# loicmagne/tinynerf

Measured on AMD Instinct MI355X. Metric: ray-samples/sec (K-Planes training step: sampler + render fwd + bwd + Adam), higher is better.
Workload: dtype f32 (f16x2-split products)

## Files before the change

tinynerf_amd/csrc/b3_device.h:

```cpp
#pragma once
#include "tn_common.h"

namespace tn {
namespace b3 {

typedef __bf16 bf16x8 __attribute__((ext_vector_type(8)));
typedef unsigned u32x4 __attribute__((ext_vector_type(4)));
typedef float f32x16 __attribute__((ext_vector_type(16)));

struct Op { u32x4 hi, mid, lo; };

__device__ __forceinline__ void split2(float a, float b, unsigned &hi, unsigned &mid, unsigned &lo) {
    const unsigned ha = __float_as_uint(a) & 0xffff0000u, hb = __float_as_uint(b) & 0xffff0000u;
    const float ra = a - __uint_as_float(ha), rb = b - __uint_as_float(hb);
    const unsigned ma = __float_as_uint(ra) & 0xffff0000u, mb = __float_as_uint(rb) & 0xffff0000u;
    const float la = ra - __uint_as_float(ma), lb = rb - __uint_as_float(mb);
    hi = __builtin_amdgcn_perm(hb, ha, 0x07060302u);
    mid = __builtin_amdgcn_perm(mb, ma, 0x07060302u);
    lo = __builtin_amdgcn_perm(__float_as_uint(lb), __float_as_uint(la), 0x07060302u);
}

__device__ __forceinline__ Op split8(const float (&v)[8]) {
    Op o;
#pragma unroll
    for (int p = 0; p < 4; ++p) {
        unsigned a, b, c;
        split2(v[2 * p], v[2 * p + 1], a, b, c);
        o.hi[p] = a; o.mid[p] = b; o.lo[p] = c;
    }
    return o;
}

__device__ __forceinline__ f32x16 mfma16(const u32x4 &a, const u32x4 &b, f32x16 c) {
    return __builtin_amdgcn_mfma_f32_32x32x16_bf16(__builtin_bit_cast(bf16x8, a), __builtin_bit_cast(bf16x8, b), c, 0, 0, 0);
}

__device__ __forceinline__ f32x16 mfma6(const Op &A, const Op &B, f32x16 acc) {
    acc = mfma16(A.lo, B.hi, acc);
    acc = mfma16(A.hi, B.lo, acc);
    acc = mfma16(A.mid, B.mid, acc);
    acc = mfma16(A.mid, B.hi, acc);
    acc = mfma16(A.hi, B.mid, acc);
    acc = mfma16(A.hi, B.hi, acc);
    return acc;
}

}
}
```

tinynerf_amd/csrc/mlp_wgrad_rc.hip:

```cpp
#include "mlp_stage.h"
#include "mlp_f2_heads.h"
#include "b3_device.h"
#include <algorithm>

#ifndef TN_RC_SB
#define TN_RC_SB
#endif
#ifdef TN_PHASE_TIMERS
__device__ unsigned long long tn_phase_cycles_rc[16];
#define TN_PTR_BEGIN unsigned long long ptr_ = __builtin_amdgcn_s_memtime();
#define TN_PTR(k) { __builtin_amdgcn_sched_barrier(0); const unsigned long long n_ = __builtin_amdgcn_s_memtime(); if (tn::lane_id() == 0) atomicAdd(&tn_phase_cycles_rc[k], n_ - ptr_); ptr_ = __builtin_amdgcn_s_memtime(); __builtin_amdgcn_sched_barrier(0); }
extern "C" int tn_debug_phase_cycles_rc(unsigned long long *out, int reset) {
    hipMemcpyFromSymbol(out, HIP_SYMBOL(tn_phase_cycles_rc), sizeof(unsigned long long) * 16);
    if (reset) { unsigned long long z[16] = {}; hipMemcpyToSymbol(HIP_SYMBOL(tn_phase_cycles_rc), z, sizeof(z)); }
    return 0;
}
#else
#define TN_PTR_BEGIN
#define TN_PTR(k)
#endif
namespace {

using tn::f32x16;
using tn::f32x4;
using namespace tn::mlp;
namespace b3 = tn::b3;

constexpr int H = 64, NH = 4;

template <int CTRL>
__device__ __forceinline__ float dpp_max(float v) {
    return fmaxf(v, __int_as_float(__builtin_amdgcn_update_dpp(0, __float_as_int(v), CTRL, 0xf, 0xf, true)));
}
__device__ __forceinline__ float wave_max(float m) {
    m = dpp_max<0xB1>(m);
    m = dpp_max<0x4E>(m);
    m = dpp_max<0x141>(m);
    m = dpp_max<0x128>(m);
    const auto r16 = __builtin_amdgcn_permlane16_swap(__float_as_uint(m), __float_as_uint(m), false, false);
    m = fmaxf(__uint_as_float(r16[0]), __uint_as_float(r16[1]));
    const auto r32 = __builtin_amdgcn_permlane32_swap(__float_as_uint(m), __float_as_uint(m), false, false);
    return fmaxf(__uint_as_float(r32[0]), __uint_as_float(r32[1]));
}

__device__ __forceinline__ void load_block_f(const float *__restrict__ rows, int i, int h, float (&v)[16]) {
    const f32x4 *p = reinterpret_cast<const f32x4 *>(rows + i * 32 + 4 * h);
#pragma unroll
    for (int q = 0; q < 4; ++q) {
        const f32x4 t = p[2 * q];
        v[4 * q] = t[0]; v[4 * q + 1] = t[1]; v[4 * q + 2] = t[2]; v[4 * q + 3] = t[3];
    }
}

__device__ __forceinline__ void split_block(const float (&v)[16], b3::Op (&op)[2]) {
    const float a[8] = {v[0], v[1], v[2], v[3], v[4], v[5], v[6], v[7]};
    const float b[8] = {v[8], v[9], v[10], v[11], v[12], v[13], v[14], v[15]};
    op[0] = b3::split8(a);
    op[1] = b3::split8(b);
}

struct WOp { u32x4h a0h, a0l, a1h, a1l; };
__device__ __forceinline__ WOp load_w(const _Float16 *__restrict__ Wh, int plane, int stride, int j, int h, int b) {
    const _Float16 *p0 = Wh + j * stride + 16 * b + 8 * h, *p1 = p0 + 32 * stride;
    WOp w;
    w.a0h = *reinterpret_cast<const u32x4h *>(p0); w.a0l = *reinterpret_cast<const u32x4h *>(p0 + plane);
    w.a1h = *reinterpret_cast<const u32x4h *>(p1); w.a1l = *reinterpret_cast<const u32x4h *>(p1 + plane);
    return w;
}
template <bool S>
__device__ __forceinline__ void mma_sf(const WOp &w, const u32x4h &bh, const u32x4h &bl, f32x16 (&accS)[2], f32x16 (&accF)[2], bool first = false) {
    const f32x16 z = {0.f, 0.f, 0.f, 0.f, 0.f, 0.f, 0.f, 0.f, 0.f, 0.f, 0.f, 0.f, 0.f, 0.f, 0.f, 0.f};
    if constexpr (S) {
        accS[0] = mfma_f16(w.a0l, bh, first ? z : accS[0]);
        accS[1] = mfma_f16(w.a1l, bh, first ? z : accS[1]);
    }
    accF[0] = mfma_f16(bh, w.a0l, first ? z : accF[0]);
    accF[1] = mfma_f16(bh, w.a1l, first ? z : accF[1]);
    if constexpr (S) {
        accS[0] = mfma_f16(w.a0h, bl, accS[0]);
        accS[1] = mfma_f16(w.a1h, bl, accS[1]);
    }
    accF[0] = mfma_f16(bl, w.a0h, accF[0]);
    accF[1] = mfma_f16(bl, w.a1h, accF[1]);
    if constexpr (S) {
        accS[0] = mfma_f16(w.a0h, bh, accS[0]);
        accS[1] = mfma_f16(w.a1h, bh, accS[1]);
    }
    accF[0] = mfma_f16(bh, w.a0h, accF[0]);
    accF[1] = mfma_f16(bh, w.a1h, accF[1]);
}

__device__ __forceinline__ void zero2(f32x16 (&a)[2]) {
#pragma unroll
    for (int ob = 0; ob < 2; ++ob)
#pragma unroll
        for (int r = 0; r < 16; ++r) a[ob][r] = 0.0f;
}

struct RcArgs {
    MlpArgs a, b;
    const float *x, *aux;
    const float *ws_a, *ws_b;
    float *gW[5], *gB[5];
    float *gWs, *gBs;
    int64_t n;
};

template <int WPB, bool AUX, int OA, int OB, int NGA, int NBA>
__device__ __forceinline__ void wgrad_rc_body(const RcArgs &p, const float *__restrict__ ldsa, const float *__restrict__ ldsb, float *__restrict__ ,
                                              const float *__restrict__ px, const float *__restrict__ paux, const int *__restrict__ paidx,
                                              const float *__restrict__ pws_a, const float *__restrict__ pws_b)
{
    const int lane = tn::lane_id(), j_ = lane & 31, h_ = lane >> 5;
    const int wave = __builtin_amdgcn_readfirstlane(threadIdx.x >> 6);
    const int64_t n = p.n, n_tiles = (n + 31) >> 5;
    const int Rta = stash_rows(H, NH, 0), Rtb = stash_rows(H, 1, 0);
    constexpr int nga = NGA, nba = NBA;
    constexpr bool has_aux = AUX;

    f32x16 acc[3][2][2];
#pragma unroll
    for (int l = 0; l < 3; ++l)
#pragma unroll
        for (int tn_ = 0; tn_ < 2; ++tn_)
#pragma unroll
            for (int tk = 0; tk < 2; ++tk)
#pragma unroll
                for (int r = 0; r < 16; ++r) acc[l][tn_][tk][r] = 0.0f;
    float db[3][2] = {{0.f, 0.f}, {0.f, 0.f}, {0.f, 0.f}};
    float dwo[OA][2], dws[OB][2], dbo[OA], dbs[OB];
#pragma unroll
    for (int o = 0; o < OA; ++o) { dwo[o][0] = dwo[o][1] = 0.f; dbo[o] = 0.f; }
#pragma unroll
    for (int o = 0; o < OB; ++o) { dws[o][0] = dws[o][1] = 0.f; dbs[o] = 0.f; }

    f32x4 fr[12], av[8];
    auto fetch_x = [&](int64_t t) {
        int64_t r = t * 32 + j_;
        r = r < n ? r : n - 1;
        const float *xr = px + r * 96 + 4 * h_;
#pragma unroll
        for (int g = 0; g < 12; ++g) fr[g] = *reinterpret_cast<const f32x4 *>(xr + 8 * g);
    };
    int aidx = 0;
    auto fetch_aidx = [&](int64_t t) {
        int64_t r = t * 32 + j_;
        r = r < n ? r : n - 1;
        if constexpr (has_aux) aidx = paidx[r];
    };
    auto fetch_aux = [&]() {
        if constexpr (has_aux) {
            const float *arow = paux + (int64_t)aidx * p.a.aux_stride + 4 * h_;
#pragma unroll
            for (int g = 0; g < 8; ++g) av[g] = *reinterpret_cast<const f32x4 *>(arow + 8 * (g < nga ? g : nga - 1));
        }
    };
    {
        const int64_t t0 = (int64_t)blockIdx.x * WPB + wave;
        fetch_aidx(t0 < n_tiles ? t0 : n_tiles - 1);
        fetch_aux();
        fetch_x(t0 < n_tiles ? t0 : n_tiles - 1);
    }
    float gqa[2][16], gqb[2][16];
    for (int64_t tile = (int64_t)blockIdx.x * WPB + wave; tile < n_tiles; tile += (int64_t)gridDim.x * WPB) {
        int j = j_, h = h_;
        asm volatile("" : "+v"(j), "+v"(h));
        const float *wsa = pws_a + tile * (int64_t)(Rta * 32);
        const float *wsb = pws_b + tile * (int64_t)(Rtb * 32);
        const _Float16 *W0 = reinterpret_cast<const _Float16 *>(ldsa + p.a.w_off[0]);
        const int plane0 = p.a.f2_plane[0], st0 = p.a.stride[0];
        const int64_t tile_next = tile + (int64_t)gridDim.x * WPB < n_tiles ? tile + (int64_t)gridDim.x * WPB : n_tiles - 1;
        fetch_aidx(tile_next);
        TN_PTR_BEGIN

        f32x16 accS[2], accF[2], actS[2], actF[2];
        if constexpr (has_aux) {
            WOp w = load_w(W0, plane0, st0, j, h, 6);
            float m = 0.0f;
#pragma unroll
            for (int g = 0; g < 8; ++g) m = fmaxf(fmaxf(m, fmaxf(fabsf(av[g][0]), fabsf(av[g][1]))), fmaxf(fabsf(av[g][2]), fabsf(av[g][3])));
            float s_a, inv_a;
            f2_scales(wave_max(m), s_a, inv_a);
#pragma unroll
            for (int ba = 0; ba < nba; ++ba) {
                const WOp wn = load_w(W0, plane0, st0, j, h, 6 + (ba + 1 < nba ? ba + 1 : ba));
                const float v[8] = {av[2 * ba][0], av[2 * ba][1], av[2 * ba][2], av[2 * ba][3], av[2 * ba + 1][0], av[2 * ba + 1][1], av[2 * ba + 1][2], av[2 * ba + 1][3]};
                u32x4h bh, bl;
                f2_split8(v, s_a, bh, bl);
                mma_sf<true>(w, bh, bl, accS, accF, ba == 0);
                TN_RC_SB
                w = wn;
            }
            const float ca = inv_a * ldsa[p.a.f2_scale + 1];
#pragma unroll
            for (int ob = 0; ob < 2; ++ob) {
#pragma unroll
                for (int r = 0; r < 16; ++r) { actS[ob][r] = accS[ob][r] * ca; actF[ob][r] = accF[ob][r] * ca; }
            }
        } else {
            zero2(actS); zero2(actF);
        }
        TN_RC_SB
        TN_PTR(0)
        u32x4h xbh[6], xbl[6];
        float inv_x;
        {
            float m = 0.0f;
#pragma unroll
            for (int g = 0; g < 12; ++g) m = fmaxf(fmaxf(m, fmaxf(fabsf(fr[g][0]), fabsf(fr[g][1]))), fmaxf(fabsf(fr[g][2]), fabsf(fr[g][3])));
            float s_x;
            f2_scales(wave_max(m), s_x, inv_x);
#pragma unroll
            for (int b = 0; b < 6; ++b) {
                const float v[8] = {fr[2 * b][0], fr[2 * b][1], fr[2 * b][2], fr[2 * b][3], fr[2 * b + 1][0], fr[2 * b + 1][1], fr[2 * b + 1][2], fr[2 * b + 1][3]};
                f2_split8(v, s_x, xbh[b], xbl[b]);
            }
        }
        TN_RC_SB
        TN_PTR(1)
        load_block_f(wsa + (int64_t)((NH + 1) * H) * 32, j, h, gqa[0]);
        load_block_f(wsa + (int64_t)((NH + 1) * H + 32) * 32, j, h, gqa[1]);
        {
            WOp w = load_w(W0, plane0, st0, j, h, 0);
#pragma unroll
            for (int b = 0; b < 6; ++b) {
                const WOp wn = load_w(W0, plane0, st0, j, h, b + 1 < 6 ? b + 1 : b);
                mma_sf<true>(w, xbh[b], xbl[b], accS, accF, b == 0);
                TN_RC_SB
                w = wn;
            }
            const float cx = inv_x * ldsa[p.a.f2_scale + 1];
#pragma unroll
            for (int ob = 0; ob < 2; ++ob) {
                const f32x16 bias = tn::bias_tile(ldsa + p.a.b_off[0], ob, h);
                const float bl_ = ldsa[p.a.b_off[0] + 32 * ob + j];
#pragma unroll
                for (int r = 0; r < 16; ++r) {
                    actS[ob][r] = fmaf(accS[ob][r], cx, actS[ob][r]) + bias[r];
                    actF[ob][r] = fmaf(accF[ob][r], cx, actF[ob][r]) + bl_;
                }
                actS[ob] = tn::relu16(actS[ob]);
                actF[ob] = tn::relu16(actF[ob]);
            }
        }
        TN_RC_SB
        TN_PTR(2)
        {
            const _Float16 *W0s = reinterpret_cast<const _Float16 *>(ldsb + p.b.w_off[0]);
            const int pls = p.b.f2_plane[0], sts = p.b.stride[0];
            float gs[OB][16];
#pragma unroll
            for (int o = 0; o < OB; ++o) load_block_f(wsb + 2 * H * 32, o, h, gs[o]);
            WOp w = load_w(W0s, pls, sts, j, h, 0);
#pragma unroll
            for (int b = 0; b < 6; ++b) {
                const WOp wn = load_w(W0s, pls, sts, j, h, b + 1 < 6 ? b + 1 : b);
                mma_sf<false>(w, xbh[b], xbl[b], accS, accF, b == 0);
                TN_RC_SB
                w = wn;
            }
            const float c = inv_x * ldsb[p.b.f2_scale + 1];
#pragma unroll
            for (int ob = 0; ob < 2; ++ob) {
                const float bias = ldsb[p.b.b_off[0] + 32 * ob + j];
#pragma unroll
                for (int r = 0; r < 16; ++r) accF[ob][r] = fmaf(accF[ob][r], c, bias);
                accF[ob] = tn::relu16(accF[ob]);
            }
#pragma unroll
            for (int o = 0; o < OB; ++o) {
                float s0 = 0.f, s1 = 0.f, sg = 0.f;
#pragma unroll
                for (int r = 0; r < 16; ++r) { s0 = fmaf(gs[o][r], accF[0][r], s0); s1 = fmaf(gs[o][r], accF[1][r], s1); sg += gs[o][r]; }
                dws[o][0] += s0; dws[o][1] += s1; dbs[o] += sg;
            }
        }
        TN_RC_SB
        TN_PTR(3)

        float go[OA][16];
#pragma unroll
        for (int l = 1; l <= 3; ++l) {
            const _Float16 *Wl = reinterpret_cast<const _Float16 *>(ldsa + p.a.w_off[l]);
            const int plane = p.a.f2_plane[l], stride = p.a.stride[l];
            float (&gq)[2][16] = (l == 2) ? gqb : gqa;
            if (l < 3) {
                float (&gn)[2][16] = (l == 1) ? gqb : gqa;
                load_block_f(wsa + (int64_t)((NH + l + 1) * H) * 32, j, h, gn[0]);
                load_block_f(wsa + (int64_t)((NH + l + 1) * H + 32) * 32, j, h, gn[1]);
            }
            {
                b3::Op HB[2][2];
#pragma unroll
                for (int tk = 0; tk < 2; ++tk) {
                    float v[16];
#pragma unroll
                    for (int r = 0; r < 16; ++r) v[r] = actF[tk][r];
                    split_block(v, HB[tk]);
                }
#pragma unroll
                for (int tn_ = 0; tn_ < 2; ++tn_) {
                    float sg = 0.f;
#pragma unroll
                    for (int r = 0; r < 16; ++r) sg += gq[tn_][r];
                    db[l - 1][tn_] += sg;
                    b3::Op GA[2];
                    split_block(gq[tn_], GA);
#pragma unroll
                    for (int c = 0; c < 2; ++c)
#pragma unroll
                        for (int tk = 0; tk < 2; ++tk) acc[l - 1][tn_][tk] = b3::mfma6(GA[c], HB[tk][c], acc[l - 1][tn_][tk]);
                    TN_RC_SB
                }
            }
            TN_PTR(3 + l)
            if (l == 1) fetch_aux();
            if (l == 3) {
#pragma unroll
                for (int o = 0; o < OA; ++o) load_block_f(wsa + 2 * NH * H * 32, o, h, go[o]);
                fetch_x(tile_next);
            }
            WOp w = load_w(Wl, plane, stride, j, h, 0);
            float m = 0.0f;
#pragma unroll
            for (int kb = 0; kb < 2; ++kb)
#pragma unroll
                for (int r = 0; r < 16; ++r) m = fmaxf(m, actS[kb][r]);
            float s, inv;
            f2_scales(wave_max(m), s, inv);
#pragma unroll
            for (int b = 0; b < 4; ++b) {
                const WOp wn = load_w(Wl, plane, stride, j, h, b + 1 < 4 ? b + 1 : b);
                float v[8];
#pragma unroll
                for (int e = 0; e < 8; ++e) v[e] = actS[b >> 1][8 * (b & 1) + e];
                u32x4h bh, bl;
                f2_split8(v, s, bh, bl);
                if (l < 3) mma_sf<true>(w, bh, bl, accS, accF, b == 0);
                else mma_sf<false>(w, bh, bl, accS, accF, b == 0);
                TN_RC_SB
                w = wn;
            }
            const float c = inv * ldsa[p.a.f2_scale + 2 * l + 1];
#pragma unroll
            for (int ob = 0; ob < 2; ++ob) {
                const float bl_ = ldsa[p.a.b_off[l] + 32 * ob + j];
#pragma unroll
                for (int r = 0; r < 16; ++r) actF[ob][r] = fmaf(accF[ob][r], c, bl_);
                actF[ob] = tn::relu16(actF[ob]);
                if (l < 3) {
                    const f32x16 bias = tn::bias_tile(ldsa + p.a.b_off[l], ob, h);
#pragma unroll
                    for (int r = 0; r < 16; ++r) actS[ob][r] = fmaf(accS[ob][r], c, bias[r]);
                    actS[ob] = tn::relu16(actS[ob]);
                }
            }
            TN_RC_SB
            TN_PTR(6 + l)
        }
#pragma unroll
        for (int o = 0; o < OA; ++o) {
            float s0 = 0.f, s1 = 0.f, sg = 0.f;
#pragma unroll
            for (int r = 0; r < 16; ++r) { s0 = fmaf(go[o][r], actF[0][r], s0); s1 = fmaf(go[o][r], actF[1][r], s1); sg += go[o][r]; }
            dwo[o][0] += s0; dwo[o][1] += s1; dbo[o] += sg;
        }
        TN_PTR(10)
    }

    const int i = j_, h = h_;
#pragma unroll
    for (int l = 0; l < 3; ++l) {
#pragma unroll
        for (int tn_ = 0; tn_ < 2; ++tn_) {
#pragma unroll
            for (int tk = 0; tk < 2; ++tk) {
                tn::pin16(acc[l][tn_][tk]);
#pragma unroll
                for (int r = 0; r < 16; ++r) {
                    const int nn = 32 * tn_ + (r & 3) + 8 * (r >> 2) + 4 * h;
                    atomicAdd(&p.gW[l + 1][nn * H + 32 * tk + i], acc[l][tn_][tk][r]);
                }
            }
            float s = db[l][tn_];
            s += __shfl_xor(s, 32, 64);
            if (h == 0) atomicAdd(&p.gB[l + 1][32 * tn_ + i], s);
        }
    }
#pragma unroll
    for (int o = 0; o < OA; ++o) {
#pragma unroll
        for (int tk = 0; tk < 2; ++tk) {
            float s = dwo[o][tk];
            s += __shfl_xor(s, 32, 64);
            if (h == 0) atomicAdd(&p.gW[4][o * H + 32 * tk + i], s);
        }
        float s = dbo[o];
        s += __shfl_xor(s, 32, 64);
        if (lane == 0) atomicAdd(&p.gB[4][o], s);
    }
#pragma unroll
    for (int o = 0; o < OB; ++o) {
#pragma unroll
        for (int tk = 0; tk < 2; ++tk) {
            float s = dws[o][tk];
            s += __shfl_xor(s, 32, 64);
            if (h == 0) atomicAdd(&p.gWs[o * H + 32 * tk + i], s);
        }
        float s = dbs[o];
        s += __shfl_xor(s, 32, 64);
        if (lane == 0) atomicAdd(&p.gBs[o], s);
    }
}

template <int WPB, bool AUX, int OA, int OB, int NGA, int NBA>
__global__ __launch_bounds__(WPB * 64) void wgrad_rc_kernel(RcArgs p)
{
    extern __shared__ __attribute__((aligned(16))) float lds[];
    stage_weights_f2(p.a, lds);
    stage_weights_f2(p.b, lds + p.a.lds_floats);
    wgrad_rc_body<WPB, AUX, OA, OB, NGA, NBA>(p, lds, lds + p.a.lds_floats, nullptr, p.x, p.aux,
                                              p.a.aux_index, p.ws_a, p.ws_b);
}

struct FlArgs {
    const float *x, *aux;
    const int *aux_index;
    int aux_stride, pe, K0_a, K0_b;
    const float *ws_a, *ws_b;
    int rt_a, rt_b, g0_a, g0_b;
    float *gW0, *gB0, *gW0s, *gB0s;
    int64_t n;
};

constexpr int FL_RS = 36;
constexpr int FL_IN = 96, FL_AW = 56;
constexpr int FL_BUF = 128 * FL_RS + 32 * FL_IN + 32 * FL_AW;

__global__ __launch_bounds__(512) void wgrad_first_kernel(FlArgs p)
{
    extern __shared__ __attribute__((aligned(16))) float lds[];
    constexpr int NW = 8, NCH = 4;
    constexpr int g_chunks = 128 * 8, x_chunks = 32 * FL_IN / 4;
    const int lane = tn::lane_id(), i_ = lane & 31, h_ = lane >> 5;
    const int wave = __builtin_amdgcn_readfirstlane(threadIdx.x >> 6);
    const int64_t n = p.n, n_tiles = (n + 31) >> 5;
    const bool colour = wave < 5;
    const int tk = colour ? wave : wave - 5;
    f32x16 acc[2];
    float dbacc[2] = {0.f, 0.f};
#pragma unroll
    for (int m = 0; m < 2; ++m)
#pragma unroll
        for (int r = 0; r < 16; ++r) acc[m][r] = 0.0f;
    f32x4 pre[NCH];
    f32x4 preA = {0.f, 0.f, 0.f, 0.f};
    int aidx = 0;
    auto prefetch = [&](int64_t tile, int64_t tile_after) {
        const f32x4 *sa = reinterpret_cast<const f32x4 *>(p.ws_a + tile * (int64_t)p.rt_a * 32 + (int64_t)p.g0_a * 32);
        const f32x4 *sb = reinterpret_cast<const f32x4 *>(p.ws_b + tile * (int64_t)p.rt_b * 32 + (int64_t)p.g0_b * 32);
        const int64_t x0 = tile * 32 * (int64_t)FL_IN;
        const int64_t xlast = n * (int64_t)FL_IN - 4;
#pragma unroll
        for (int k = 0; k < NCH; ++k) {
            const int c = threadIdx.x + k * NW * 64;
            int64_t e = x0 + 4 * (int64_t)(c - g_chunks);
            e = e < 0 ? 0 : (e > xlast ? xlast : e);
            const f32x4 *px = reinterpret_cast<const f32x4 *>(p.x + e);
            const f32x4 *pg = c < 512 ? sa + c : sb + ((c - 512) & 511);
            pre[k] = *(c < g_chunks ? pg : px);
        }
        {
            const int s_ = (threadIdx.x >> 4) & 31, part = threadIdx.x & 15;
            preA = *reinterpret_cast<const f32x4 *>(p.aux + (int64_t)aidx * p.aux_stride + (4 * part < FL_AW ? 4 * part : 0));
            int64_t r_ = tile_after * 32 + s_;
            r_ = r_ < n ? r_ : n - 1;
            aidx = p.aux_index[r_];
        }
    };
    float *dummy = lds + 2 * FL_BUF;
    auto commit = [&](float *buf) {
        float *ldsX = buf + 128 * FL_RS, *ldsA = ldsX + 32 * FL_IN;
#pragma unroll
        for (int k = 0; k < NCH; ++k) {
            const int c = threadIdx.x + k * NW * 64;
            float *dst = c < g_chunks ? buf + (c >> 3) * FL_RS + (c & 7) * 4 : (c < g_chunks + x_chunks ? ldsX + 4 * (c - g_chunks) : dummy);
            *reinterpret_cast<f32x4 *>(dst) = pre[k];
        }
        const int s_ = threadIdx.x >> 4, part = threadIdx.x & 15;
        float *dst = 4 * part < FL_AW ? ldsA + s_ * FL_AW + 4 * part : dummy;
        *reinterpret_cast<f32x4 *>(dst) = preA;
    };
    const int64_t last = n_tiles - 1;
    int64_t tile = blockIdx.x;
    if (tile >= n_tiles) return;
    {
        int64_t r_ = tile * 32 + ((threadIdx.x >> 4) & 31);
        r_ = r_ < n ? r_ : n - 1;
        aidx = p.aux_index[r_];
    }
    {
        const int64_t t1 = tile + gridDim.x, t2 = t1 + gridDim.x;
        prefetch(tile, t1 < last ? t1 : last);
        commit(lds);
        __syncthreads();
        prefetch(t1 < last ? t1 : last, t2 < last ? t2 : last);
    }
    int cur = 0;
    for (; tile < n_tiles; tile += gridDim.x) {
        int i = i_, h = h_;
        asm volatile("" : "+v"(i), "+v"(h));
        float *buf = lds + cur * FL_BUF;
        float *nbuf = lds + (cur ^ 1) * FL_BUF;
        const int64_t t2 = tile + 2 * (int64_t)gridDim.x, t3 = t2 + gridDim.x;
        commit(nbuf);
        prefetch(t2 < last ? t2 : last, t3 < last ? t3 : last);
        const float *ldsX = buf + 128 * FL_RS, *ldsA = ldsX + 32 * FL_IN;
        {
            const int grow = colour ? 0 : 64;
            const f32x4 *g0 = reinterpret_cast<const f32x4 *>(buf + (grow + i) * FL_RS + 16 * h);
            const f32x4 *g1 = reinterpret_cast<const f32x4 *>(buf + (grow + 32 + i) * FL_RS + 16 * h);
            const int q = 32 * tk + i;
            const bool xcol = q < FL_IN;
            const int ac = q - FL_IN < FL_AW ? q - FL_IN : FL_AW - 1;
            const float *cp = xcol ? ldsX + 16 * h * FL_IN + q : ldsA + 16 * h * FL_AW + (ac < 0 ? 0 : ac);
            const int cstride = xcol ? FL_IN : FL_AW;
            float gs0 = 0.f, gs1 = 0.f;
#pragma unroll
            for (int c = 0; c < 2; ++c) {
                const f32x4 ga = g0[2 * c], gb = g0[2 * c + 1], gc = g1[2 * c], gd = g1[2 * c + 1];
                float xv[8];
#pragma unroll
                for (int u = 0; u < 8; ++u) xv[u] = cp[(8 * c + u) * cstride];
                const float v0[8] = {ga[0], ga[1], ga[2], ga[3], gb[0], gb[1], gb[2], gb[3]};
                const float v1[8] = {gc[0], gc[1], gc[2], gc[3], gd[0], gd[1], gd[2], gd[3]};
                const b3::Op XB = b3::split8(xv);
                acc[0] = b3::mfma6(b3::split8(v0), XB, acc[0]);
                acc[1] = b3::mfma6(b3::split8(v1), XB, acc[1]);
                gs0 += ((ga[0] + ga[1]) + (ga[2] + ga[3])) + ((gb[0] + gb[1]) + (gb[2] + gb[3]));
                gs1 += ((gc[0] + gc[1]) + (gc[2] + gc[3])) + ((gd[0] + gd[1]) + (gd[2] + gd[3]));
            }
            if (tk == 0) { dbacc[0] += gs0; dbacc[1] += gs1; }
        }
        __syncthreads();
        cur ^= 1;
    }
    const int i = i_, h = h_;
    const int q = 32 * tk + i;
    int col; bool ok;
    float *gW; int ldw;
    if (colour) { gW = p.gW0; ldw = p.K0_a; ok = q < FL_IN || q - FL_IN < p.pe; col = q < FL_IN ? p.pe + q : q - FL_IN; }
    else { gW = p.gW0s; ldw = p.K0_b; ok = true; col = q; }
#pragma unroll
    for (int m = 0; m < 2; ++m) {
        tn::pin16(acc[m]);
#pragma unroll
        for (int r = 0; r < 16; ++r) {
            const int nn = 32 * m + (r & 3) + 8 * (r >> 2) + 4 * h;
            if (ok) atomicAdd(&gW[(int64_t)nn * ldw + col], acc[m][r]);
        }
        if (tk == 0) {
            float s = dbacc[m];
            s += __shfl_xor(s, 32, 64);
            if (h == 0) atomicAdd(&(colour ? p.gB0 : p.gB0s)[32 * m + i], s);
        }
    }
}

}

static bool lean_pair_ok(const tn_mlp_desc *d, const tn_mlp_desc *p)
{
    const bool f2 = (d->flags & TN_MLP_F16X2) && (p->flags & TN_MLP_F16X2);
    return f2 && d->n_layers == 5 && p->n_layers == 2 && d->in_dim == 96 && p->in_dim == 96 && d->encoding == TN_ENC_AUX_CAT &&
           p->encoding == TN_ENC_NONE && d->dims[0] == 147 && d->dims[1] == 64 && d->dims[2] == 64 && d->dims[3] == 64 &&
           d->dims[4] == 64 && d->dims[5] == 3 && p->dims[0] == 96 && p->dims[1] == 64 && p->dims[2] == 1 &&
           d->aux_stride >= FL_AW && (d->aux_stride & 3) == 0;
}

extern "C" int tn_mlp_lean_supported(const tn_mlp_desc *desc, const tn_mlp_desc *partner)
{
    return desc && partner && lean_pair_ok(desc, partner);
}

static int lean_plan(RcArgs &p, const tn_mlp_desc *desc, const tn_mlp_desc *partner, const float *x, const float *aux, int64_t n,
                     float *const *gw, float *const *gb, float *const *gws, float *const *gbs, const float *ws_a, const float *ws_b)
{
    TN_REQUIRE(desc && partner && x && gw && gb && gws && gbs && ws_a && ws_b, TN_E_NULL, "tn_mlp_wgrad_lean_pair: null pointer");
    int Ha = 0, Hb = 0;
    if (int rc = plan(desc, p.a, Ha)) return rc;
    if (int rc = plan(partner, p.b, Hb)) return rc;
    TN_REQUIRE(lean_pair_ok(desc, partner), TN_E_CONFIG, "TN_MLP_LEAN: the reference's decoders (run.py:133-139) as f16x2 heads (TN_MLP_F16X2): "
                                                         "colour 147 -> 64 x 4 -> 3 on [per-ray table (51), x (96)], sigma 96 -> 64 -> 1");
    TN_REQUIRE(aux && ((uintptr_t)aux & 15) == 0 && p.a.aux_index, TN_E_NULL, "TN_MLP_LEAN: aux table (16-byte aligned) and aux_index are required");
    TN_REQUIRE((((uintptr_t)x | (uintptr_t)ws_a | (uintptr_t)ws_b) & 15) == 0, TN_E_ALIGN, "TN_MLP_LEAN: x / workspaces must be 16-byte aligned");
    if (n <= 0) return TN_OK;
    for (int l = 0; l < 5; ++l) TN_REQUIRE(gw[l] && gb[l], TN_E_NULL, "TN_MLP_LEAN: null gradient pointer");
    TN_REQUIRE(gws[0] && gbs[0] && gws[1] && gbs[1], TN_E_NULL, "TN_MLP_LEAN: null gradient pointer");
    plan_f2(p.a, 64);
    plan_f2(p.b, 64);
    TN_REQUIRE(((size_t)p.a.lds_floats + (size_t)p.b.lds_floats) * 4 <= (size_t)LDS_LIMIT_BYTES, TN_E_CONFIG, "TN_MLP_LEAN: weights do not fit LDS");
    return TN_OK;
}

extern "C" __attribute__((visibility("hidden"))) int tn_mlp_wgrad_lean_check(const tn_mlp_desc *desc, const tn_mlp_desc *partner, const float *x,
                                                                             const float *aux, int64_t n, float *const *gw, float *const *gb,
                                                                             float *const *gws, float *const *gbs, const float *ws_a,
                                                                             const float *ws_b)
{
    RcArgs p;
    return lean_plan(p, desc, partner, x, aux, n, gw, gb, gws, gbs, ws_a, ws_b);
}

extern "C" int tn_mlp_wgrad_lean_pair(const tn_mlp_desc *desc, const tn_mlp_desc *partner, const float *x, const float *aux, int64_t n,
                                      float *const *gw, float *const *gb, float *const *gws, float *const *gbs, const float *ws_a,
                                      const float *ws_b, void *stream)
{
    RcArgs p;
    if (int rc = lean_plan(p, desc, partner, x, aux, n, gw, gb, gws, gbs, ws_a, ws_b)) return rc;
    if (n <= 0) return TN_OK;
    hipStream_t s = (hipStream_t)stream;
    FlArgs f;
    f.x = x; f.aux = aux; f.aux_index = p.a.aux_index; f.aux_stride = p.a.aux_stride;
    f.pe = p.a.K0 - p.a.in_dim;
    f.ws_a = ws_a; f.ws_b = ws_b;
    f.rt_a = stash_rows(H, NH, 0); f.rt_b = stash_rows(H, 1, 0);
    f.g0_a = NH * H; f.g0_b = H;
    f.K0_a = p.a.K0; f.K0_b = p.b.K0;
    f.gW0 = gw[0]; f.gB0 = gb[0]; f.gW0s = gws[0]; f.gB0s = gbs[0];
    f.n = n;
    const size_t lds1 = (2 * (size_t)FL_BUF + 16) * 4;
    if (int rc = launch(wgrad_first_kernel, 8, lds1, grid_blocks(n, 1, 256 * 2), s, "wgrad_first_kernel", f)) return rc;
    p.x = x; p.aux = aux; p.ws_a = ws_a; p.ws_b = ws_b; p.n = n;
    for (int l = 0; l < 5; ++l) { p.gW[l] = gw[l]; p.gB[l] = gb[l]; }
    p.gWs = gws[1]; p.gBs = gbs[1];
    constexpr int WPB = 4;
    const size_t lds_bytes = ((size_t)p.a.lds_floats + (size_t)p.b.lds_floats) * 4;
    return launch(wgrad_rc_kernel<WPB, true, 3, 1, 7, 4>, WPB, lds_bytes, grid_blocks(n, WPB, 256), s, "wgrad_rc_kernel", p);
}
```

Measured before the change: 345.4 million.

## Pin wgrad accumulators to AGPR tiles, interleave MFMA chains, use 32-bit indices

The weight-gradient MFMA accumulation now goes through inline asm that pins each of the 12 accumulator tiles to a fixed AGPR range, and the 3-way split products for the two k-tiles are interleaved so consecutive MFMAs write independent accumulators. Per-layer f2 scales are hoisted out of the tile loop into scalar registers, and the tile and row index arithmetic moves from 64-bit to 32-bit, with a new host check capping n. The aim is to cut accumulator spills and copies, MFMA dependency stalls and scalar/VALU index overhead, at the cost of hand-managed register allocation and s_nop padding that may conflict with the compiler's own scheduling.

```diff
diff --git a/tinynerf_amd/csrc/b3_device.h b/tinynerf_amd/csrc/b3_device.h
--- a/tinynerf_amd/csrc/b3_device.h
+++ b/tinynerf_amd/csrc/b3_device.h
@@ -45,5 +45,15 @@
     return acc;
 }
 
+template <typename F>
+__device__ __forceinline__ void mfma6_ip2(const Op &A, const Op &B0, const Op &B1, F &&mma) {
+    mma(0, A.lo, B0.hi);   mma(1, A.lo, B1.hi);
+    mma(0, A.hi, B0.lo);   mma(1, A.hi, B1.lo);
+    mma(0, A.mid, B0.mid); mma(1, A.mid, B1.mid);
+    mma(0, A.mid, B0.hi);  mma(1, A.mid, B1.hi);
+    mma(0, A.hi, B0.mid);  mma(1, A.hi, B1.mid);
+    mma(0, A.hi, B0.hi);   mma(1, A.hi, B1.hi);
+}
+
 }
 }
diff --git a/tinynerf_amd/csrc/mlp_wgrad_rc.hip b/tinynerf_amd/csrc/mlp_wgrad_rc.hip
--- a/tinynerf_amd/csrc/mlp_wgrad_rc.hip
+++ b/tinynerf_amd/csrc/mlp_wgrad_rc.hip
@@ -90,6 +90,17 @@
     accF[1] = mfma_f16(bh, w.a1h, accF[1]);
 }
 
+#define TN_RC_TILE(t, lo, hi) \
+    case t: asm("s_nop 1\n\tv_mfma_f32_32x32x16_bf16 %0, %2, %3, %0" : "={a[" #lo ":" #hi "]}"(c) : "0"(c), "v"(a), "v"(b)); asm("" : "+a"(c)); break;
+__device__ __forceinline__ void mfma16_tile(int t, const b3::u32x4 &a, const b3::u32x4 &b, f32x16 &c) {
+    switch (t) {
+        TN_RC_TILE(0, 0, 15) TN_RC_TILE(1, 16, 31) TN_RC_TILE(2, 32, 47) TN_RC_TILE(3, 48, 63)
+        TN_RC_TILE(4, 64, 79) TN_RC_TILE(5, 80, 95) TN_RC_TILE(6, 96, 111) TN_RC_TILE(7, 112, 127)
+        TN_RC_TILE(8, 128, 143) TN_RC_TILE(9, 144, 159) TN_RC_TILE(10, 160, 175) TN_RC_TILE(11, 176, 191)
+    }
+}
+#undef TN_RC_TILE
+
 __device__ __forceinline__ void zero2(f32x16 (&a)[2]) {
 #pragma unroll
     for (int ob = 0; ob < 2; ++ob)
@@ -112,8 +123,10 @@
                                               const float *__restrict__ pws_a, const float *__restrict__ pws_b)
 {
     const int lane = tn::lane_id(), j_ = lane & 31, h_ = lane >> 5;
+    int j = j_, h = h_;
     const int wave = __builtin_amdgcn_readfirstlane(threadIdx.x >> 6);
-    const int64_t n = p.n, n_tiles = (n + 31) >> 5;
+    const int n_last = (int)p.n - 1;
+    const int n_tiles = (int)((p.n + 31) >> 5), tile_step = (int)gridDim.x * WPB;
     const int Rta = stash_rows(H, NH, 0), Rtb = stash_rows(H, 1, 0);
     constexpr int nga = NGA, nba = NBA;
     constexpr bool has_aux = AUX;
@@ -135,41 +148,42 @@
     for (int o = 0; o < OB; ++o) { dws[o][0] = dws[o][1] = 0.f; dbs[o] = 0.f; }
 
     f32x4 fr[12], av[8];
-    auto fetch_x = [&](int64_t t) {
-        int64_t r = t * 32 + j_;
-        r = r < n ? r : n - 1;
-        const float *xr = px + r * 96 + 4 * h_;
+    auto fetch_x = [&](int t) {
+        const int r = min(t * 32 + j, n_last);
+        const float *xr = px + (int64_t)r * 96 + 4 * h;
 #pragma unroll
         for (int g = 0; g < 12; ++g) fr[g] = *reinterpret_cast<const f32x4 *>(xr + 8 * g);
     };
     int aidx = 0;
-    auto fetch_aidx = [&](int64_t t) {
-        int64_t r = t * 32 + j_;
-        r = r < n ? r : n - 1;
+    auto fetch_aidx = [&](int t) {
+        const int r = min(t * 32 + j, n_last);
         if constexpr (has_aux) aidx = paidx[r];
     };
     auto fetch_aux = [&]() {
         if constexpr (has_aux) {
-            const float *arow = paux + (int64_t)aidx * p.a.aux_stride + 4 * h_;
+            const float *arow = paux + (int64_t)aidx * p.a.aux_stride + 4 * h;
 #pragma unroll
             for (int g = 0; g < 8; ++g) av[g] = *reinterpret_cast<const f32x4 *>(arow + 8 * (g < nga ? g : nga - 1));
         }
     };
     {
-        const int64_t t0 = (int64_t)blockIdx.x * WPB + wave;
+        const int t0 = (int)blockIdx.x * WPB + wave;
         fetch_aidx(t0 < n_tiles ? t0 : n_tiles - 1);
         fetch_aux();
         fetch_x(t0 < n_tiles ? t0 : n_tiles - 1);
     }
+    float wsc[NH], wsc_s;
+#pragma unroll
+    for (int l = 0; l < NH; ++l) wsc[l] = __uint_as_float(__builtin_amdgcn_readfirstlane(__float_as_uint(ldsa[p.a.f2_scale + 2 * l + 1])));
+    wsc_s = __uint_as_float(__builtin_amdgcn_readfirstlane(__float_as_uint(ldsb[p.b.f2_scale + 1])));
     float gqa[2][16], gqb[2][16];
-    for (int64_t tile = (int64_t)blockIdx.x * WPB + wave; tile < n_tiles; tile += (int64_t)gridDim.x * WPB) {
-        int j = j_, h = h_;
+    for (int tile = (int)blockIdx.x * WPB + wave; tile < n_tiles; tile += tile_step) {
         asm volatile("" : "+v"(j), "+v"(h));
         const float *wsa = pws_a + tile * (int64_t)(Rta * 32);
         const float *wsb = pws_b + tile * (int64_t)(Rtb * 32);
         const _Float16 *W0 = reinterpret_cast<const _Float16 *>(ldsa + p.a.w_off[0]);
         const int plane0 = p.a.f2_plane[0], st0 = p.a.stride[0];
-        const int64_t tile_next = tile + (int64_t)gridDim.x * WPB < n_tiles ? tile + (int64_t)gridDim.x * WPB : n_tiles - 1;
+        const int tile_next = n_tiles - tile > tile_step ? tile + tile_step : n_tiles - 1;
         fetch_aidx(tile_next);
         TN_PTR_BEGIN
 
@@ -191,7 +205,7 @@
                 TN_RC_SB
                 w = wn;
             }
-            const float ca = inv_a * ldsa[p.a.f2_scale + 1];
+            const float ca = inv_a * wsc[0];
 #pragma unroll
             for (int ob = 0; ob < 2; ++ob) {
 #pragma unroll
@@ -229,7 +243,7 @@
                 TN_RC_SB
                 w = wn;
             }
-            const float cx = inv_x * ldsa[p.a.f2_scale + 1];
+            const float cx = inv_x * wsc[0];
 #pragma unroll
             for (int ob = 0; ob < 2; ++ob) {
                 const f32x16 bias = tn::bias_tile(ldsa + p.a.b_off[0], ob, h);
@@ -259,7 +273,7 @@
                 TN_RC_SB
                 w = wn;
             }
-            const float c = inv_x * ldsb[p.b.f2_scale + 1];
+            const float c = inv_x * wsc_s;
 #pragma unroll
             for (int ob = 0; ob < 2; ++ob) {
                 const float bias = ldsb[p.b.b_off[0] + 32 * ob + j];
@@ -308,8 +322,9 @@
                     split_block(gq[tn_], GA);
 #pragma unroll
                     for (int c = 0; c < 2; ++c)
-#pragma unroll
-                        for (int tk = 0; tk < 2; ++tk) acc[l - 1][tn_][tk] = b3::mfma6(GA[c], HB[tk][c], acc[l - 1][tn_][tk]);
+                        b3::mfma6_ip2(GA[c], HB[0][c], HB[1][c], [&](int tk, const b3::u32x4 &a, const b3::u32x4 &b) {
+                            mfma16_tile(4 * (l - 1) + 2 * tn_ + tk, a, b, acc[l - 1][tn_][tk]);
+                        });
                     TN_RC_SB
                 }
             }
@@ -341,7 +356,7 @@
                 TN_RC_SB
                 w = wn;
             }
-            const float c = inv * ldsa[p.a.f2_scale + 2 * l + 1];
+            const float c = inv * wsc[l];
 #pragma unroll
             for (int ob = 0; ob < 2; ++ob) {
                 const float bl_ = ldsa[p.a.b_off[l] + 32 * ob + j];
@@ -368,7 +383,7 @@
         TN_PTR(10)
     }
 
-    const int i = j_, h = h_;
+    const int i = j;
 #pragma unroll
     for (int l = 0; l < 3; ++l) {
 #pragma unroll
@@ -397,7 +412,7 @@
         }
         float s = dbo[o];
         s += __shfl_xor(s, 32, 64);
-        if (lane == 0) atomicAdd(&p.gB[4][o], s);
+        if ((j | h) == 0) atomicAdd(&p.gB[4][o], s);
     }
 #pragma unroll
     for (int o = 0; o < OB; ++o) {
@@ -409,7 +424,7 @@
         }
         float s = dbs[o];
         s += __shfl_xor(s, 32, 64);
-        if (lane == 0) atomicAdd(&p.gBs[o], s);
+        if ((j | h) == 0) atomicAdd(&p.gBs[o], s);
     }
 }
 
@@ -595,6 +610,7 @@
     TN_REQUIRE(aux && ((uintptr_t)aux & 15) == 0 && p.a.aux_index, TN_E_NULL, "TN_MLP_LEAN: aux table (16-byte aligned) and aux_index are required");
     TN_REQUIRE((((uintptr_t)x | (uintptr_t)ws_a | (uintptr_t)ws_b) & 15) == 0, TN_E_ALIGN, "TN_MLP_LEAN: x / workspaces must be 16-byte aligned");
     if (n <= 0) return TN_OK;
+    TN_REQUIRE(n < ((int64_t)1 << 31) - 32, TN_E_CONFIG, "TN_MLP_LEAN: n must be below 2^31 - 32 (32-bit sample indices)");
     for (int l = 0; l < 5; ++l) TN_REQUIRE(gw[l] && gb[l], TN_E_NULL, "TN_MLP_LEAN: null gradient pointer");
     TN_REQUIRE(gws[0] && gbs[0] && gws[1] && gbs[1], TN_E_NULL, "TN_MLP_LEAN: null gradient pointer");
     plan_f2(p.a, 64);
```

New measurement: 341.5 million. 0.989x the previous value.
